# igormq/aes-lac-2018

Hardware: AMD Instinct MI355X
Metric: train frames/sec, DeepSpeech2 5xBiGRU-800 (higher is better)
Workload: dtype f32

## Files before the change

aes-lac-2018_amd/csrc/bn.hip:

```cpp
#include "ds2_common.h"

namespace {

constexpr int NPART = 64;

template <int MODE>
__global__ __launch_bounds__(256) void bn2d_reduce_kernel(const float* __restrict__ x, const float* __restrict__ dy,
                                                          const float* __restrict__ mean_invstd,
                                                          const float* __restrict__ gamma,
                                                          const float* __restrict__ beta, int B, int C, int inner,
                                                          double* __restrict__ part) {
    const int c = blockIdx.y, p = blockIdx.x, tid = threadIdx.x;
    const int chunks = (inner + 1023) / 1024;
    const int items = B * chunks;
    float mu = 0.f, is = 0.f, ga = 0.f, be = 0.f;
    if (MODE == 1) {
        mu = mean_invstd[c];
        is = mean_invstd[C + c];
        ga = gamma[c];
        be = beta[c];
    }
    float s0 = 0.f, s1 = 0.f;
    for (int it = p; it < items; it += NPART) {
        const int b = it / chunks, ch = it % chunks;
        const size_t base = ((size_t)b * C + c) * inner;
        const int i0 = ch * 1024;
#pragma unroll
        for (int u = 0; u < 4; ++u) {
            const int i = i0 + u * 256 + tid;
            if (i < inner) {
                const float v = x[base + i];
                if (MODE == 0) {
                    s0 += v;
                    s1 += v * v;
                } else {
                    const float xh = (v - mu) * is;
                    const float y = ga * xh + be;
                    const float g = (y > 0.f && y < 20.f) ? dy[base + i] : 0.f;
                    s0 += g;
                    s1 += g * xh;
                }
            }
        }
    }
    double d0 = wave_sum_d((double)s0), d1 = wave_sum_d((double)s1);
    __shared__ double sm[4][2];
    if ((tid & 63) == 0) {
        sm[tid >> 6][0] = d0;
        sm[tid >> 6][1] = d1;
    }
    __syncthreads();
    if (tid == 0) {
        part[((size_t)c * NPART + p) * 2 + 0] = sm[0][0] + sm[1][0] + sm[2][0] + sm[3][0];
        part[((size_t)c * NPART + p) * 2 + 1] = sm[0][1] + sm[1][1] + sm[2][1] + sm[3][1];
    }
}

template <int MODE>
__global__ __launch_bounds__(256) void bn2d_reduce_vec_kernel(const float* __restrict__ x, const float* __restrict__ dy,
                                                              const float* __restrict__ mean_invstd,
                                                              const float* __restrict__ gamma,
                                                              const float* __restrict__ beta, int B, int C, int inner,
                                                              double* __restrict__ part) {
    const int c = blockIdx.y, p = blockIdx.x, tid = threadIdx.x;
    const int chunks = (inner + 1023) / 1024;
    const int items = B * chunks;
    float mu = 0.f, is = 0.f, ga = 0.f, be = 0.f;
    if (MODE == 1) {
        mu = mean_invstd[c];
        is = mean_invstd[C + c];
        ga = gamma[c];
        be = beta[c];
    }
    float s0 = 0.f, s1 = 0.f;
    auto take = [&](float v, float g) {
        if (MODE == 0) {
            s0 += v;
            s1 += v * v;
        } else {
            const float xh = (v - mu) * is;
            const float y = ga * xh + be;
            const float gm = (y > 0.f && y < 20.f) ? g : 0.f;
            s0 += gm;
            s1 += gm * xh;
        }
    };
// ... 3 lines not shown
        const int h = min((int)((4 - (base & 3)) & 3), inner);
        const int nq = (inner - h) >> 2;
        const int q = ch * 256 + tid;
        if (q < nq) {
            const f32x4 v = *reinterpret_cast<const f32x4*>(x + base + h + 4 * (size_t)q);
            f32x4 g = {0.f, 0.f, 0.f, 0.f};
            if (MODE == 1) g = *reinterpret_cast<const f32x4*>(dy + base + h + 4 * (size_t)q);
#pragma unroll
            for (int e = 0; e < 4; ++e) take(v[e], g[e]);
        }
        if (ch == 0) {
            const int tail0 = h + 4 * nq, e = tid < 4 ? tid : tail0 + tid - 4;
            if ((tid < h) || (tid >= 4 && tid < 8 && e < inner)) take(x[base + e], MODE == 1 ? dy[base + e] : 0.f);
        }
    }
    double d0 = wave_sum_d((double)s0), d1 = wave_sum_d((double)s1);
    __shared__ double sm[4][2];
    if ((tid & 63) == 0) {
        sm[tid >> 6][0] = d0;
        sm[tid >> 6][1] = d1;
    }
    __syncthreads();
    if (tid == 0) {
        part[((size_t)c * NPART + p) * 2 + 0] = sm[0][0] + sm[1][0] + sm[2][0] + sm[3][0];
        part[((size_t)c * NPART + p) * 2 + 1] = sm[0][1] + sm[1][1] + sm[2][1] + sm[3][1];
    }
}

template <int MODE>
__global__ __launch_bounds__(256) void bn1d_reduce_kernel(const float* __restrict__ xa, const float* __restrict__ xb,
                                                          const float* __restrict__ dy,
                                                          const float* __restrict__ mean_invstd, int rows, int F,
                                                          double* __restrict__ part) {
    const int p = blockIdx.x, tid = threadIdx.x;
    const int col = blockIdx.y * 64 + (tid & 63), ry = tid >> 6;
    float mu = 0.f, is = 0.f;
    if (MODE == 1 && col < F) {
        mu = mean_invstd[col];
        is = mean_invstd[F + col];
    }
    float s0 = 0.f, s1 = 0.f;
    if (col < F) {
        for (int r = p * 4 + ry; r < rows; r += NPART * 4) {
            const size_t o = (size_t)r * F + col;
            float v = xa[o];
            if (xb) v += xb[o];
            if (MODE == 0) {
                s0 += v;
                s1 += v * v;
            } else {
                const float g = dy[o];
                s0 += g;
                s1 += g * (v - mu) * is;
            }
        }
    }
    __shared__ float sm[4][64][2];
    sm[ry][tid & 63][0] = s0;
    sm[ry][tid & 63][1] = s1;
    __syncthreads();
    if (ry == 0 && col < F) {
        const int l = tid & 63;
        const double d0 = (double)sm[0][l][0] + (double)sm[1][l][0] + (double)sm[2][l][0] + (double)sm[3][l][0];
        const double d1 = (double)sm[0][l][1] + (double)sm[1][l][1] + (double)sm[2][l][1] + (double)sm[3][l][1];
        part[((size_t)col * NPART + p) * 2 + 0] = d0;
        part[((size_t)col * NPART + p) * 2 + 1] = d1;
    }
}

__global__ __launch_bounds__(64) void bn_finalize_stats_kernel(const double* __restrict__ part, int C, double count,
                                                               float eps, float momentum, int use_running,
                                                               float* __restrict__ running_mean,
                                                               float* __restrict__ running_var,
                                                               float* __restrict__ mean_invstd) {
    const int c = blockIdx.x, lane = threadIdx.x;
    if (use_running) {
        if (lane == 0) {
            mean_invstd[c] = running_mean[c];
            mean_invstd[C + c] = (float)(1.0 / sqrt((double)running_var[c] + (double)eps));
        }
        return;
    }
    double s0 = part[((size_t)c * NPART + lane) * 2 + 0];
    double s1 = part[((size_t)c * NPART + lane) * 2 + 1];
    s0 = wave_sum_d(s0);
    s1 = wave_sum_d(s1);
    if (lane == 0) {
        const double mean = s0 / count;
        double var = s1 / count - mean * mean;
        if (var < 0.0) var = 0.0;
        mean_invstd[c] = (float)mean;
        mean_invstd[C + c] = (float)(1.0 / sqrt(var + (double)eps));
        if (running_mean) {
            const double unb = count > 1.0 ? var * count / (count - 1.0) : var;
            running_mean[c] = (float)((1.0 - momentum) * running_mean[c] + momentum * mean);
            running_var[c] = (float)((1.0 - momentum) * running_var[c] + momentum * unb);
        }
    }
}

__global__ __launch_bounds__(64) void bn_finalize_bwd_kernel(const double* __restrict__ part, int C, double count,
                                                             float* __restrict__ dgamma, float* __restrict__ dbeta,
                                                             float* __restrict__ coef) {
    const int c = blockIdx.x, lane = threadIdx.x;
    double s0 = part[((size_t)c * NPART + lane) * 2 + 0];
    double s1 = part[((size_t)c * NPART + lane) * 2 + 1];
    s0 = wave_sum_d(s0);
    s1 = wave_sum_d(s1);
    if (lane == 0) {
        dbeta[c] = (float)s0;
        dgamma[c] = (float)s1;
        coef[c] = (float)(s0 / count);
        coef[C + c] = (float)(s1 / count);
    }
}

__global__ __launch_bounds__(256) void bn2d_apply_kernel(const float* __restrict__ x,
                                                         const float* __restrict__ mean_invstd,
                                                         const float* __restrict__ gamma,
                                                         const float* __restrict__ beta, int C, int inner,
                                                         float* __restrict__ y) {
    const int bc = blockIdx.y, c = bc % C;
    const float sc = gamma[c] * mean_invstd[C + c];
    const float sh = beta[c] - mean_invstd[c] * sc;
    const size_t base = (size_t)bc * inner;
    for (int i = blockIdx.x * 256 + threadIdx.x; i < inner; i += gridDim.x * 256) {
        const float v = x[base + i] * sc + sh;
        y[base + i] = fminf(fmaxf(v, 0.f), 20.f);
    }
}

__global__ __launch_bounds__(256) void bn2d_apply_tbf_kernel(const float* __restrict__ x,
                                                             const float* __restrict__ mean_invstd,
                                                             const float* __restrict__ gamma,
                                                             const float* __restrict__ beta, int B, int C, int D,
                                                             int T, float* __restrict__ y) {
    __shared__ float tile[32][33];
// ... 155 lines not shown
            } else {
                const f32x4 g = dy[o];
                s0 += g;
                s1 += g * (v - mu) * is;
            }
        }
    }
    __shared__ f32x4 sm[4][64][2];
    sm[ry][tid & 63][0] = s0;
    sm[ry][tid & 63][1] = s1;
    __syncthreads();
    if (ry == 0 && cq < F4) {
        const int l = tid & 63;
#pragma unroll
        for (int e = 0; e < 4; ++e) {
            const double d0 = (double)sm[0][l][0][e] + (double)sm[1][l][0][e] + (double)sm[2][l][0][e] + (double)sm[3][l][0][e];
            const double d1 = (double)sm[0][l][1][e] + (double)sm[1][l][1][e] + (double)sm[2][l][1][e] + (double)sm[3][l][1][e];
            part[((size_t)(4 * cq + e) * NPART + p) * 2 + 0] = d0;
            part[((size_t)(4 * cq + e) * NPART + p) * 2 + 1] = d1;
        }
    }
}

__global__ __launch_bounds__(256) void bn1d_apply_vec_kernel(const f32x4* __restrict__ xa, const f32x4* __restrict__ xb,
                                                             const float* __restrict__ mean_invstd,
                                                             const float* __restrict__ gamma,
                                                             const float* __restrict__ beta, size_t n4, int F4,
                                                             f32x4* __restrict__ y) {
    const size_t stride = (size_t)gridDim.x * 256;
    for (size_t i = (size_t)blockIdx.x * 256 + threadIdx.x; i < n4; i += stride) {
        const int c = 4 * (int)(i % F4);
        f32x4 v = xa[i];
        if (xb) v += xb[i];
        const f32x4 sc = *reinterpret_cast<const f32x4*>(gamma + c) * *reinterpret_cast<const f32x4*>(mean_invstd + 4 * F4 + c);
        y[i] = (v - *reinterpret_cast<const f32x4*>(mean_invstd + c)) * sc + *reinterpret_cast<const f32x4*>(beta + c);
    }
}

__global__ __launch_bounds__(256) void bn1d_bwd_apply_vec_kernel(const f32x4* __restrict__ xa, const f32x4* __restrict__ xb,
                                                                 const f32x4* __restrict__ dy,
                                                                 const float* __restrict__ mean_invstd,
                                                                 const float* __restrict__ gamma,
                                                                 const float* __restrict__ coef, size_t n4, int F4,
                                                                 f32x4* __restrict__ dx) {
    const size_t stride = (size_t)gridDim.x * 256;
    const int F = 4 * F4;
    for (size_t i = (size_t)blockIdx.x * 256 + threadIdx.x; i < n4; i += stride) {
        const int c = 4 * (int)(i % F4);
        f32x4 v = xa[i];
        if (xb) v += xb[i];
        const f32x4 is = *reinterpret_cast<const f32x4*>(mean_invstd + F + c);
        const f32x4 xh = (v - *reinterpret_cast<const f32x4*>(mean_invstd + c)) * is;
        dx[i] = *reinterpret_cast<const f32x4*>(gamma + c) * is *
                (dy[i] - *reinterpret_cast<const f32x4*>(coef + c) - xh * *reinterpret_cast<const f32x4*>(coef + F + c));
    }
}

inline bool aligned16(const void* p) { return ((uintptr_t)p & 15) == 0; }
inline bool vec4_ok(int F, const void* a, const void* b, const void* c, const void* d) {
    return (F & 3) == 0 && ((((uintptr_t)a) | ((uintptr_t)b) | ((uintptr_t)c) | ((uintptr_t)d)) & 15) == 0;
}

inline int ew_blocks(size_t n) {
    size_t b = (n + 255) / 256;
    if (b > 4096) b = 4096;
    if (b < 1) b = 1;
    return (int)b;
}

}

extern "C" size_t ds2_bn_ws_bytes(int C) { return (size_t)C * NPART * 2 * sizeof(double) + (size_t)C * 2 * sizeof(float); }

extern "C" int ds2_bn2d_stats(const float* x, int B, int C, int inner, float eps, float momentum, int use_running,
                              float* running_mean, float* running_var, float* mean_invstd, void* ws, void* stream) {
    DS2_CHECK_ARG(x && mean_invstd && ws && B > 0 && C > 0 && inner > 0);
    DS2_CHECK_ARG(!use_running || (running_mean && running_var));
    hipStream_t st = (hipStream_t)stream;
    double* part = (double*)ws;
    if (!use_running) {
        if (aligned16(x))
            hipLaunchKernelGGL((bn2d_reduce_vec_kernel<0>), dim3(NPART, C), dim3(256), 0, st, x, nullptr, nullptr, nullptr,
                               nullptr, B, C, inner, part);
        else
            hipLaunchKernelGGL((bn2d_reduce_kernel<0>), dim3(NPART, C), dim3(256), 0, st, x, nullptr, nullptr, nullptr,
                               nullptr, B, C, inner, part);
    }
    hipLaunchKernelGGL(bn_finalize_stats_kernel, dim3(C), dim3(64), 0, st, part, C, (double)B * inner, eps, momentum,
                       use_running, running_mean, running_var, mean_invstd);
    DS2_CHECK_LAUNCH();
    return DS2_OK;
}

extern "C" int ds2_bn2d_apply_htanh(const float* x, const float* mean_invstd, const float* gamma, const float* beta,
                                    int B, int C, int D, int T, int layout_tbf, float* y, void* stream) {
    DS2_CHECK_ARG(x && mean_invstd && gamma && beta && y && B > 0 && C > 0 && D > 0 && T > 0);
    hipStream_t st = (hipStream_t)stream;
    if (layout_tbf) {
        DS2_CHECK_ARG(B <= 65535);
        dim3 grid(ds2_cdiv(T, 32), ds2_cdiv(C * D, 32), B);
        hipLaunchKernelGGL(bn2d_apply_tbf_kernel, grid, dim3(256), 0, st, x, mean_invstd, gamma, beta, B, C, D, T, y);
    } else {
        const int inner = D * T;
        if (aligned16(x) && aligned16(y)) {
            dim3 grid(min(ds2_cdiv(inner, 1024), 64), B * C);
            hipLaunchKernelGGL(bn2d_apply_vec_kernel, grid, dim3(256), 0, st, x, mean_invstd, gamma, beta, C, inner, y);
        } else {
            dim3 grid(min(ds2_cdiv(inner, 256), 64), B * C);
            hipLaunchKernelGGL(bn2d_apply_kernel, grid, dim3(256), 0, st, x, mean_invstd, gamma, beta, C, inner, y);
        }
    }
    DS2_CHECK_LAUNCH();
    return DS2_OK;
}

extern "C" int ds2_bn2d_htanh_bwd(const float* x, const float* dy, const float* mean_invstd, const float* gamma,
                                  const float* beta, int B, int C, int D, int T, float* dx, float* dgamma,
                                  float* dbeta, void* ws, void* stream) {
    DS2_CHECK_ARG(x && dy && mean_invstd && gamma && beta && dx && dgamma && dbeta && ws);
    DS2_CHECK_ARG(B > 0 && C > 0 && D > 0 && T > 0);
    hipStream_t st = (hipStream_t)stream;
    const int inner = D * T;
    double* part = (double*)ws;
    float* coef = (float*)(part + (size_t)C * NPART * 2);
    const bool vec = aligned16(x) && aligned16(dy) && aligned16(dx);
    if (vec)
        hipLaunchKernelGGL((bn2d_reduce_vec_kernel<1>), dim3(NPART, C), dim3(256), 0, st, x, dy, mean_invstd, gamma, beta,
                           B, C, inner, part);
    else
        hipLaunchKernelGGL((bn2d_reduce_kernel<1>), dim3(NPART, C), dim3(256), 0, st, x, dy, mean_invstd, gamma, beta, B,
                           C, inner, part);
    hipLaunchKernelGGL(bn_finalize_bwd_kernel, dim3(C), dim3(64), 0, st, part, C, (double)B * inner, dgamma, dbeta,
                       coef);
    if (vec) {
        dim3 grid(min(ds2_cdiv(inner, 1024), 64), B * C);
        hipLaunchKernelGGL(bn2d_bwd_apply_vec_kernel, grid, dim3(256), 0, st, x, dy, mean_invstd, gamma, beta, coef, C,
                           inner, dx);
    } else {
        dim3 grid(min(ds2_cdiv(inner, 256), 64), B * C);
        hipLaunchKernelGGL(bn2d_bwd_apply_kernel, grid, dim3(256), 0, st, x, dy, mean_invstd, gamma, beta, coef, C, inner,
                           dx);
    }
    DS2_CHECK_LAUNCH();
    return DS2_OK;
}

extern "C" int ds2_bn1d_stats(const float* xa, const float* xb, int rows, int F, float eps, float momentum,
                              int use_running, float* running_mean, float* running_var, float* mean_invstd, void* ws,
                              void* stream) {
    DS2_CHECK_ARG(xa && mean_invstd && ws && rows > 0 && F > 0);
    DS2_CHECK_ARG(!use_running || (running_mean && running_var));
    hipStream_t st = (hipStream_t)stream;
    double* part = (double*)ws;
    if (!use_running) {
        if (vec4_ok(F, xa, xb, nullptr, nullptr))
            hipLaunchKernelGGL((bn1d_reduce_vec_kernel<0>), dim3(NPART, ds2_cdiv(F / 4, 64)), dim3(256), 0, st,
                               (const f32x4*)xa, (const f32x4*)xb, nullptr, nullptr, rows, F, part);
        else
            hipLaunchKernelGGL((bn1d_reduce_kernel<0>), dim3(NPART, ds2_cdiv(F, 64)), dim3(256), 0, st, xa, xb, nullptr,
                               nullptr, rows, F, part);
    }
    hipLaunchKernelGGL(bn_finalize_stats_kernel, dim3(F), dim3(64), 0, st, part, F, (double)rows, eps, momentum,
                       use_running, running_mean, running_var, mean_invstd);
    DS2_CHECK_LAUNCH();
    return DS2_OK;
}

extern "C" int ds2_bn1d_apply(const float* xa, const float* xb, const float* mean_invstd, const float* gamma,
                              const float* beta, int rows, int F, float* y, void* stream) {
    DS2_CHECK_ARG(xa && mean_invstd && gamma && beta && y && rows > 0 && F > 0);
    const size_t n = (size_t)rows * F;
    if (vec4_ok(F, xa, xb, y, gamma) && vec4_ok(F, beta, mean_invstd, nullptr, nullptr))
        hipLaunchKernelGGL(bn1d_apply_vec_kernel, dim3(ew_blocks(n / 4)), dim3(256), 0, (hipStream_t)stream,
                           (const f32x4*)xa, (const f32x4*)xb, mean_invstd, gamma, beta, n / 4, F / 4, (f32x4*)y);
    else
        hipLaunchKernelGGL(bn1d_apply_kernel, dim3(ew_blocks(n)), dim3(256), 0, (hipStream_t)stream, xa, xb,
                           mean_invstd, gamma, beta, n, F, y);
    DS2_CHECK_LAUNCH();
    return DS2_OK;
}

extern "C" int ds2_bn1d_bwd(const float* xa, const float* xb, const float* dy, const float* mean_invstd,
                            const float* gamma, int rows, int F, float* dx, float* dgamma, float* dbeta, void* ws,
                            void* stream) {
    DS2_CHECK_ARG(xa && dy && mean_invstd && gamma && dx && dgamma && dbeta && ws && rows > 0 && F > 0);
    hipStream_t st = (hipStream_t)stream;
    double* part = (double*)ws;
    float* coef = (float*)(part + (size_t)F * NPART * 2);
    const bool vec = vec4_ok(F, xa, xb, dy, dx) && vec4_ok(F, gamma, mean_invstd, nullptr, nullptr);
    if (vec)
        hipLaunchKernelGGL((bn1d_reduce_vec_kernel<1>), dim3(NPART, ds2_cdiv(F / 4, 64)), dim3(256), 0, st,
                           (const f32x4*)xa, (const f32x4*)xb, (const f32x4*)dy, mean_invstd, rows, F, part);
    else
        hipLaunchKernelGGL((bn1d_reduce_kernel<1>), dim3(NPART, ds2_cdiv(F, 64)), dim3(256), 0, st, xa, xb, dy,
                           mean_invstd, rows, F, part);
    hipLaunchKernelGGL(bn_finalize_bwd_kernel, dim3(F), dim3(64), 0, st, part, F, (double)rows, dgamma, dbeta, coef);
    const size_t n = (size_t)rows * F;
    if (vec)
        hipLaunchKernelGGL(bn1d_bwd_apply_vec_kernel, dim3(ew_blocks(n / 4)), dim3(256), 0, st, (const f32x4*)xa,
                           (const f32x4*)xb, (const f32x4*)dy, mean_invstd, gamma, coef, n / 4, F / 4, (f32x4*)dx);
    else
        hipLaunchKernelGGL(bn1d_bwd_apply_kernel, dim3(ew_blocks(n)), dim3(256), 0, st, xa, xb, dy, mean_invstd, gamma,
                           coef, n, F, dx);
    DS2_CHECK_LAUNCH();
    return DS2_OK;
}
```

aes-lac-2018_amd/csrc/conv_split.hip:

```cpp
#include <stdlib.h>

#include <type_traits>

#include "split_bf16.h"

namespace {

constexpr int G_OOB = 0x7FFFFFF0;
constexpr int SPARE = 4;

struct GatherGeom {
    int M;
    int ngroups, npairs;
    int pair_stride, D;
    int row_len, rows_per_b;
    int a_base, a_b_stride, a_row_stride;
    int o_base, o_b_stride, o_row_stride, o_col_stride;
    int frows;
};

template <int NPROD, int NT>
__global__ __launch_bounds__(256, 2) void conv2_gather_kernel(const float* __restrict__ A, unsigned int a_bytes,
                                                              const int* __restrict__ tap_off,
                                                              const unsigned int* __restrict__ Wp, unsigned int w_bytes,
// ... 143 lines not shown
                    *c = acc[i][r] + bv;
            }
        }
}

__host__ __device__ inline int tap_groups(int nrows) { return 3 * (nrows / 2) + 2 * (nrows & 1); }
__device__ __forceinline__ void tap_slot(int nrows, int gq, int j, int& row, int& tap) {
    const int pairs = nrows >> 1;
    if (gq < 3 * pairs) {
        const int pr = gq / 3, w = gq - pr * 3;
        if (w < 2) {
            row = 2 * pr + w;
            tap = j;
        } else {
            row = 2 * pr + (j >> 2);
            tap = 8 + (j & 3);
        }
    } else {
        row = nrows - 1;
        tap = gq == 3 * pairs ? j : (j < 4 ? 8 + j : 11);
    }
    if (tap > 10) row = -1;
}
__global__ void conv2_split_prepare_kernel(const float* __restrict__ w, int mode, int nrows, int line, int spare,
                                           int* __restrict__ tap_off, unsigned int* __restrict__ Wp) {
    const int ng = tap_groups(nrows);
    const int i = blockIdx.x * 256 + threadIdx.x;
    if (i < (ng + spare) * 2) {
        const int gq = min(i >> 1, ng - 1);
        int row, tap;
        tap_slot(nrows, gq, (i & 1) * 4, row, tap);
        if (row < 0) tap_slot(nrows, gq, 0, row, tap);
        tap_off[i] = (mode == 0 ? row : 10 - row) * line + tap;
    }
    const int total = (16 * ng + spare) * 32 * 2 * 4;
    if (i >= total) return;
    const int jp = i & 3, half = (i >> 2) & 1, n = (i >> 3) & 31, step = i >> 8;
    const int cp = step / ng, gq = step - cp * ng;
    float v[2] = {0.f, 0.f};
    if (cp < 16) {
        const int c = 2 * cp + half;
#pragma unroll
        for (int e = 0; e < 2; ++e) {
            int row, tap;
            tap_slot(nrows, gq, jp * 2 + e, row, tap);
            if (row >= 0)
                v[e] = mode == 0 ? w[((n * 32 + c) * 21 + row) * 11 + tap]
                                 : w[((c * 32 + n) * 21 + 2 * row + (mode - 1)) * 11 + 10 - tap];
        }
    }
    unsigned int p1, p2, p3;
    split3(v[0], v[1], p1, p2, p3);
    unsigned int* dst = Wp + ((size_t)step * 3 * 32 * 16 + (n * 16 + half * 8 + jp * 2)) / 2;
    dst[0] = p1;
    dst[(32 * 16) / 2] = p2;
    dst[2 * (32 * 16) / 2] = p3;
}

__global__ __launch_bounds__(256) void conv2_pad_dout_kernel(const float* __restrict__ dy, int B, int T,
                                                             float* __restrict__ dyp) {
    const int TP = T + 20, nrows = B * 32 * 41;
    for (int r = blockIdx.x; r < nrows; r += gridDim.x) {
        const int bc = r / 41, fo = r - bc * 41 - 10;
        float* dst = dyp + (size_t)r * TP;
        if (fo < 0 || fo >= 21) {
            for (int tc = threadIdx.x; tc < TP; tc += 256) dst[tc] = 0.f;
        } else {
            const float* src = dy + ((size_t)bc * 21 + fo) * T - 10;
            for (int tc = threadIdx.x; tc < TP; tc += 256) dst[tc] = (tc >= 10 && tc < T + 10) ? src[tc] : 0.f;
        }
    }
}

int conv_split_mode() {
    const char* e = getenv("DS2_CONV_SPLIT");
    const int v = e ? atoi(e) : 6;
    return (v == 6 || v == 9) ? v : 0;
}

struct GatherPlan {
    int nt, tiles, per, nsplit;
};
GatherPlan plan_gather(int M, int nstep, bool may_split) {
    static const int force_ks = ds2_tune_env("DS2_CONV_SPLIT_KS") ? atoi(ds2_tune_env("DS2_CONV_SPLIT_KS")) : 0;
    static const int force_nt = ds2_tune_env("DS2_CONV_SPLIT_NT") ? atoi(ds2_tune_env("DS2_CONV_SPLIT_NT")) : 0;
    GatherPlan p;
    const int waves64 = ds2_cdiv(M, 64);
    p.nt = force_nt > 0 ? force_nt : (waves64 >= 1536 ? 2 : 1);
    p.tiles = ds2_cdiv(M, 128 * p.nt);
    const int waves = p.tiles * 4;
    const int ks = !may_split ? 1 : (force_ks > 0 ? force_ks : (waves >= 1024 ? 1 : (waves >= 512 ? 2 : 3)));
    p.per = ds2_cdiv(nstep, ks);
    p.nsplit = ds2_cdiv(nstep, p.per);
    return p;
// ... 65 lines not shown
    const unsigned int w_bytes = (unsigned int)((NP * NG + SPARE) * 3 * 32 * 16 * 2);
    launch_gather(mode, in, (unsigned int)a_bytes, tap_off, Wp, w_bytes, bias, out, o_elems, g, nstep, nullptr, st);
    return 0;
}

size_t ds2_conv2_dgrad_split_ws_floats(int B, int t1) {
    const size_t img0 = (size_t)(16 * tap_groups(11) + SPARE) * 3 * 32 * 16 / 2, img1 = (size_t)(16 * tap_groups(10) + SPARE) * 3 * 32 * 16 / 2;
    return 1024 + img0 + img1 + (size_t)B * 32 * 41 * (t1 + 10) + 64;
}

int ds2_conv2_dgrad_split(const float* d_out, const float* weight, int B, int t1, float* d_in, void* ws, hipStream_t st) {
    const int mode = conv_split_mode();
    if (mode == 0) return 1;
    const char* on = getenv("DS2_CONV_SPLIT_DGRAD");
    static const int dgrad_min = ds2_tune_env("DS2_CONV_SPLIT_DGRAD_MIN") ? atoi(ds2_tune_env("DS2_CONV_SPLIT_DGRAD_MIN")) : 1000;
    if (on ? on[0] != '1' : (long)B * t1 < dgrad_min) return 1;
    const int T = t1 - 10, TP = T + 20;
    const unsigned long long a_bytes = 4ull * B * 32 * 41 * TP, o_elems = 1ull * B * 32 * 61 * t1;
    if (a_bytes >= 0x7FFFFFF0ull || o_elems >= 0x7FFFFFF0ull) return 1;
    const size_t img0 = (size_t)(16 * tap_groups(11) + SPARE) * 3 * 32 * 16 / 2, img1 = (size_t)(16 * tap_groups(10) + SPARE) * 3 * 32 * 16 / 2;
    int* tab = reinterpret_cast<int*>(ws);
    unsigned int* Wp[2] = {reinterpret_cast<unsigned int*>(ws) + 1024, reinterpret_cast<unsigned int*>(ws) + 1024 + img0};
    float* dyp = reinterpret_cast<float*>(ws) + 1024 + img0 + img1;
    hipLaunchKernelGGL(conv2_pad_dout_kernel, dim3(B * 32 * 41 < 8192 ? B * 32 * 41 : 8192), dim3(256), 0, st, d_out, B, T, dyp);
    bool zeroed = false;
    for (int par = 0; par < 2; ++par)
        if (plan_gather(B * (par == 0 ? 31 : 30) * t1, 16 * tap_groups(par == 0 ? 11 : 10), true).nsplit > 1) zeroed = true;
    if (zeroed) (void)hipMemsetAsync(d_in, 0, o_elems * sizeof(float), st);
    GatherGeom gg[2];
    unsigned int wb[2];
    GatherPlan pp[2];
    for (int par = 0; par < 2; ++par) {
        const int nrows = par == 0 ? 11 : 10, ng = tap_groups(nrows), RH = par == 0 ? 31 : 30;
        const int prep = (16 * ng + SPARE) * 32 * 2 * 4;
        hipLaunchKernelGGL(conv2_split_prepare_kernel, dim3(ds2_cdiv(prep, 256)), dim3(256), 0, st, weight, 1 + par, nrows, TP,
                           SPARE, tab + 512 * par, Wp[par]);
        GatherGeom& g = gg[par];
        g.M = B * RH * t1;
        g.ngroups = ng;
        g.npairs = 16;
        g.pair_stride = 2 * 41 * TP;
        g.D = 41 * TP;
        g.row_len = t1;
        g.rows_per_b = RH;
        g.a_base = 0;
        g.a_b_stride = 32 * 41 * TP;
        g.a_row_stride = TP;
        g.o_base = par * t1;
        g.o_b_stride = 32 * 61 * t1;
        g.o_row_stride = 2 * t1;
        g.o_col_stride = 61 * t1;
        const char* rows_env = getenv("DS2_CONV_DGRAD_ROWS");
        const bool rows_off = rows_env && rows_env[0] == '0';
        pp[par] = plan_gather(g.M, 16 * ng, true);
        g.frows = (!rows_off && pp[par].nsplit == 1) ? nrows : 0;
        wb[par] = (unsigned int)((16 * ng + SPARE) * 3 * 32 * 16 * 2);
    }
    const char* merge_env = getenv("DS2_CONV_DGRAD_MERGE");
    const bool merge_off = merge_env && merge_env[0] == '0';
// ... 11 lines not shown
```

aes-lac-2018_amd/csrc/optim.hip:

```cpp
#include "ds2_common.h"

namespace {

constexpr int SS_BLOCKS = 1024;

__global__ __launch_bounds__(256) void sumsq_partial_kernel(const float* __restrict__ x, size_t n4, size_t n,
                                                            double* __restrict__ part) {
    float acc = 0.f;
    double dacc = 0.0;
    const size_t stride = (size_t)gridDim.x * 256;
    int cnt = 0;
    for (size_t i = (size_t)blockIdx.x * 256 + threadIdx.x; i < n4; i += stride) {
        const f32x4 v = reinterpret_cast<const f32x4*>(x)[i];
        acc += v[0] * v[0] + v[1] * v[1] + v[2] * v[2] + v[3] * v[3];
        if (++cnt == 64) {
            dacc += (double)acc;
            acc = 0.f;
            cnt = 0;
        }
    }
    if (blockIdx.x == 0)
        for (size_t i = n4 * 4 + threadIdx.x; i < n; i += 256) acc += x[i] * x[i];
    dacc += (double)acc;
    dacc = wave_sum_d(dacc);
    __shared__ double sm[4];
    if ((threadIdx.x & 63) == 0) sm[threadIdx.x >> 6] = dacc;
    __syncthreads();
    if (threadIdx.x == 0) part[blockIdx.x] = sm[0] + sm[1] + sm[2] + sm[3];
}

__global__ __launch_bounds__(256) void sumsq_final_kernel(const double* __restrict__ part, int nparts,
                                                          double* __restrict__ out) {
    double s = 0.0;
    for (int i = threadIdx.x; i < nparts; i += 256) s += part[i];
    s = wave_sum_d(s);
    __shared__ double sm[4];
    if ((threadIdx.x & 63) == 0) sm[threadIdx.x >> 6] = s;
    __syncthreads();
    if (threadIdx.x == 0) out[0] = sm[0] + sm[1] + sm[2] + sm[3];
}

__global__ __launch_bounds__(256) void clip_sgd_kernel(float* __restrict__ p, const float* __restrict__ g,
                                                       float* __restrict__ buf, size_t n4, size_t n,
                                                       const double* __restrict__ sumsq, float grad_scale,
                                                       float max_norm, float lr, float momentum, int first_step) {
    float coef = 1.f;
    if (sumsq) {
        const float total = (float)(sqrt(sumsq[0]) * (double)fabsf(grad_scale));
        const float c = max_norm / (total + 1e-6f);
        coef = c < 1.f ? c : 1.f;
    }
// ... 45 lines not shown

extern "C" int ds2_step_stats(const float* costs, int B, const double* sumsq, const uint32_t* const* err_words,
                              int n_err, double* out, void* stream) {
    DS2_CHECK_ARG(costs && out && B > 0 && n_err >= 0 && (n_err == 0 || err_words));
    hipLaunchKernelGGL(step_stats_kernel, dim3(1), dim3(64), 0, (hipStream_t)stream, costs, B, sumsq, err_words, n_err,
                       out);
    DS2_CHECK_LAUNCH();
    return DS2_OK;
}

extern "C" size_t ds2_sumsq_ws_bytes(size_t n) {
    (void)n;
    return SS_BLOCKS * sizeof(double);
}

extern "C" int ds2_sumsq(const float* x, size_t n, double* out, void* ws, void* stream) {
    DS2_CHECK_ARG(x && out && ws && n > 0);
    DS2_CHECK_ARG(((uintptr_t)x & 15) == 0);
    hipStream_t st = (hipStream_t)stream;
    const size_t n4 = n / 4;
    int blocks = (int)((n4 + 255) / 256);
    if (blocks > SS_BLOCKS) blocks = SS_BLOCKS;
    if (blocks < 1) blocks = 1;
    hipLaunchKernelGGL(sumsq_partial_kernel, dim3(blocks), dim3(256), 0, st, x, n4, n, (double*)ws);
    hipLaunchKernelGGL(sumsq_final_kernel, dim3(1), dim3(256), 0, st, (const double*)ws, blocks, out);
    DS2_CHECK_LAUNCH();
    return DS2_OK;
}

extern "C" int ds2_clip_sgd_nesterov(float* p, const float* g, float* buf, size_t n, const double* sumsq,
                                     float grad_scale, float max_norm, float lr, float momentum, int first_step,
                                     void* stream) {
    DS2_CHECK_ARG(p && g && buf && n > 0);
    DS2_CHECK_ARG((((uintptr_t)p | (uintptr_t)g | (uintptr_t)buf) & 15) == 0);
    const size_t n4 = n / 4;
    int blocks = (int)((n4 + 255) / 256);
    if (blocks > 2048) blocks = 2048;
    if (blocks < 1) blocks = 1;
    hipLaunchKernelGGL(clip_sgd_kernel, dim3(blocks), dim3(256), 0, (hipStream_t)stream, p, g, buf, n4, n, sumsq,
                       grad_scale, max_norm, lr, momentum, first_step);
    DS2_CHECK_LAUNCH();
    return DS2_OK;
}
```

Before: 561,400.

## Fold BN and sumsq finalize into reduce kernels via last-block tickets

Batch-norm reductions and the gradient sum-of-squares now use a global atomic ticket so that the last-arriving block performs the final reduction and finalize step, removing the separate finalize kernel launches. A vectorized 1D BN reduce kernel with a transposed partial layout is added. The conv2 dgrad padding and the two weight-prepare kernels are merged into one prologue launch. All three are on by default with env opt-outs. The cost is extra atomics and fences, and the ticket slots are shared state that could collide under concurrent streams.

```diff
diff --git a/aes-lac-2018_amd/csrc/bn.hip b/aes-lac-2018_amd/csrc/bn.hip
--- a/aes-lac-2018_amd/csrc/bn.hip
+++ b/aes-lac-2018_amd/csrc/bn.hip
@@ -1,15 +1,104 @@
 #include "ds2_common.h"
+#include <atomic>
 
 namespace {
 
 constexpr int NPART = 64;
 
+constexpr int FOLD_SLOTS = 256, FOLD_GROUPS = 256;
+__device__ unsigned int g_fold_ticket[FOLD_SLOTS * FOLD_GROUPS];
+
+struct FoldTail {
+    double count;
+    float eps, momentum;
+    float *running_mean, *running_var, *mean_invstd;
+    float *dgamma, *dbeta, *coef;
+    int ticket0;
+};
+
+__device__ __forceinline__ void fold_store(double* p, double v) {
+    __hip_atomic_store(p, v, __ATOMIC_RELAXED, __HIP_MEMORY_SCOPE_AGENT);
+}
+__device__ __forceinline__ double fold_load(const double* p) {
+    return __hip_atomic_load(p, __ATOMIC_RELAXED, __HIP_MEMORY_SCOPE_AGENT);
+}
+
+__device__ __forceinline__ bool fold_last_arriver(unsigned int* ticket) {
+    __shared__ unsigned int s_last;
+    asm volatile("s_waitcnt vmcnt(0)" ::: "memory");
+    __syncthreads();
+    if (threadIdx.x == 0) {
+        const unsigned int prev = __hip_atomic_fetch_add(ticket, 1u, __ATOMIC_RELAXED, __HIP_MEMORY_SCOPE_AGENT);
+        if (prev == NPART - 1) __hip_atomic_store(ticket, 0u, __ATOMIC_RELAXED, __HIP_MEMORY_SCOPE_AGENT);
+        s_last = prev == NPART - 1;
+    }
+    __syncthreads();
+    if (!s_last) return false;
+    __builtin_amdgcn_fence(__ATOMIC_ACQUIRE, "agent");
+    return true;
+}
+
+__device__ __forceinline__ double fold_tree(const double* part, size_t stride) {
+    double a[NPART / 2];
+#pragma unroll
+    for (int l = 0; l < NPART / 2; ++l) a[l] = fold_load(part + l * stride) + fold_load(part + (l + NPART / 2) * stride);
+#pragma unroll
+    for (int o = NPART / 4; o > 0; o >>= 1)
+#pragma unroll
+        for (int l = 0; l < o; ++l) a[l] += a[l + o];
+    return a[0];
+}
+
+__device__ __forceinline__ void finalize_stats(double s0, double s1, int c, int C, double count, float eps, float momentum,
+                                               float* running_mean, float* running_var, float* mean_invstd) {
+    const double mean = s0 / count;
+    double var = s1 / count - mean * mean;
+    if (var < 0.0) var = 0.0;
+    mean_invstd[c] = (float)mean;
+    mean_invstd[C + c] = (float)(1.0 / sqrt(var + (double)eps));
+    if (running_mean) {
+        const double unb = count > 1.0 ? var * count / (count - 1.0) : var;
+        running_mean[c] = (float)((1.0 - momentum) * running_mean[c] + momentum * mean);
+        running_var[c] = (float)((1.0 - momentum) * running_var[c] + momentum * unb);
+    }
+}
+__device__ __forceinline__ void finalize_bwd(double s0, double s1, int c, int C, double count, float* dgamma, float* dbeta,
+                                             float* coef) {
+    dbeta[c] = (float)s0;
+    dgamma[c] = (float)s1;
+    coef[c] = (float)(s0 / count);
+    coef[C + c] = (float)(s1 / count);
+}
 template <int MODE>
+__device__ __forceinline__ void fold_finalize(double s0, double s1, int c, int C, const FoldTail& t) {
+    if (MODE == 0) finalize_stats(s0, s1, c, C, t.count, t.eps, t.momentum, t.running_mean, t.running_var, t.mean_invstd);
+    else finalize_bwd(s0, s1, c, C, t.count, t.dgamma, t.dbeta, t.coef);
+}
+template <int MODE>
+__device__ __forceinline__ void fold_tail_2d(const double* part, int c, int C, const FoldTail& t) {
+    if (threadIdx.x >= 64) return;
+    const int lane = threadIdx.x;
+    double s0 = fold_load(part + ((size_t)c * NPART + lane) * 2 + 0);
+    double s1 = fold_load(part + ((size_t)c * NPART + lane) * 2 + 1);
+    s0 = wave_sum_d(s0);
+    s1 = wave_sum_d(s1);
+    if (lane == 0) fold_finalize<MODE>(s0, s1, c, C, t);
+}
+__device__ __forceinline__ size_t fold_part_1d(int p, int k, int col, int F) { return ((size_t)p * 2 + k) * F + col; }
+template <int MODE>
+__device__ __forceinline__ void fold_tail_1d(const double* part, int col, int F, const FoldTail& t) {
+    if (col >= F) return;
+    const double s0 = fold_tree(part + fold_part_1d(0, 0, col, F), (size_t)2 * F);
+    const double s1 = fold_tree(part + fold_part_1d(0, 1, col, F), (size_t)2 * F);
+    fold_finalize<MODE>(s0, s1, col, F, t);
+}
+
+template <int MODE, bool FOLD>
 __global__ __launch_bounds__(256) void bn2d_reduce_kernel(const float* __restrict__ x, const float* __restrict__ dy,
                                                           const float* __restrict__ mean_invstd,
                                                           const float* __restrict__ gamma,
                                                           const float* __restrict__ beta, int B, int C, int inner,
-                                                          double* __restrict__ part) {
+                                                          double* __restrict__ part, FoldTail ft) {
     const int c = blockIdx.y, p = blockIdx.x, tid = threadIdx.x;
     const int chunks = (inner + 1023) / 1024;
     const int items = B * chunks;
@@ -51,17 +140,24 @@
     }
     __syncthreads();
     if (tid == 0) {
-        part[((size_t)c * NPART + p) * 2 + 0] = sm[0][0] + sm[1][0] + sm[2][0] + sm[3][0];
-        part[((size_t)c * NPART + p) * 2 + 1] = sm[0][1] + sm[1][1] + sm[2][1] + sm[3][1];
-    }
-}
-
-template <int MODE>
+        const double d0s = sm[0][0] + sm[1][0] + sm[2][0] + sm[3][0], d1s = sm[0][1] + sm[1][1] + sm[2][1] + sm[3][1];
+        if (FOLD) {
+            fold_store(part + ((size_t)c * NPART + p) * 2 + 0, d0s);
+            fold_store(part + ((size_t)c * NPART + p) * 2 + 1, d1s);
+        } else {
+            part[((size_t)c * NPART + p) * 2 + 0] = d0s;
+            part[((size_t)c * NPART + p) * 2 + 1] = d1s;
+        }
+    }
+    if (FOLD && fold_last_arriver(g_fold_ticket + ft.ticket0 + c)) fold_tail_2d<MODE>(part, c, C, ft);
+}
+
+template <int MODE, bool FOLD>
 __global__ __launch_bounds__(256) void bn2d_reduce_vec_kernel(const float* __restrict__ x, const float* __restrict__ dy,
                                                               const float* __restrict__ mean_invstd,
                                                               const float* __restrict__ gamma,
                                                               const float* __restrict__ beta, int B, int C, int inner,
-                                                              double* __restrict__ part) {
+                                                              double* __restrict__ part, FoldTail ft) {
     const int c = blockIdx.y, p = blockIdx.x, tid = threadIdx.x;
     const int chunks = (inner + 1023) / 1024;
     const int items = B * chunks;
@@ -111,16 +207,23 @@
     }
     __syncthreads();
     if (tid == 0) {
-        part[((size_t)c * NPART + p) * 2 + 0] = sm[0][0] + sm[1][0] + sm[2][0] + sm[3][0];
-        part[((size_t)c * NPART + p) * 2 + 1] = sm[0][1] + sm[1][1] + sm[2][1] + sm[3][1];
-    }
-}
-
-template <int MODE>
+        const double d0s = sm[0][0] + sm[1][0] + sm[2][0] + sm[3][0], d1s = sm[0][1] + sm[1][1] + sm[2][1] + sm[3][1];
+        if (FOLD) {
+            fold_store(part + ((size_t)c * NPART + p) * 2 + 0, d0s);
+            fold_store(part + ((size_t)c * NPART + p) * 2 + 1, d1s);
+        } else {
+            part[((size_t)c * NPART + p) * 2 + 0] = d0s;
+            part[((size_t)c * NPART + p) * 2 + 1] = d1s;
+        }
+    }
+    if (FOLD && fold_last_arriver(g_fold_ticket + ft.ticket0 + c)) fold_tail_2d<MODE>(part, c, C, ft);
+}
+
+template <int MODE, bool FOLD>
 __global__ __launch_bounds__(256) void bn1d_reduce_kernel(const float* __restrict__ xa, const float* __restrict__ xb,
                                                           const float* __restrict__ dy,
                                                           const float* __restrict__ mean_invstd, int rows, int F,
-                                                          double* __restrict__ part) {
+                                                          double* __restrict__ part, FoldTail ft) {
     const int p = blockIdx.x, tid = threadIdx.x;
     const int col = blockIdx.y * 64 + (tid & 63), ry = tid >> 6;
     float mu = 0.f, is = 0.f;
@@ -152,9 +255,15 @@
         const int l = tid & 63;
         const double d0 = (double)sm[0][l][0] + (double)sm[1][l][0] + (double)sm[2][l][0] + (double)sm[3][l][0];
         const double d1 = (double)sm[0][l][1] + (double)sm[1][l][1] + (double)sm[2][l][1] + (double)sm[3][l][1];
-        part[((size_t)col * NPART + p) * 2 + 0] = d0;
-        part[((size_t)col * NPART + p) * 2 + 1] = d1;
-    }
+        if (FOLD) {
+            fold_store(part + fold_part_1d(p, 0, col, F), d0);
+            fold_store(part + fold_part_1d(p, 1, col, F), d1);
+        } else {
+            part[((size_t)col * NPART + p) * 2 + 0] = d0;
+            part[((size_t)col * NPART + p) * 2 + 1] = d1;
+        }
+    }
+    if (FOLD && fold_last_arriver(g_fold_ticket + ft.ticket0 + blockIdx.y) && tid < 64) fold_tail_1d<MODE>(part, blockIdx.y * 64 + tid, F, ft);
 }
 
 __global__ __launch_bounds__(64) void bn_finalize_stats_kernel(const double* __restrict__ part, int C, double count,
@@ -174,18 +283,7 @@
     double s1 = part[((size_t)c * NPART + lane) * 2 + 1];
     s0 = wave_sum_d(s0);
     s1 = wave_sum_d(s1);
-    if (lane == 0) {
-        const double mean = s0 / count;
-        double var = s1 / count - mean * mean;
-        if (var < 0.0) var = 0.0;
-        mean_invstd[c] = (float)mean;
-        mean_invstd[C + c] = (float)(1.0 / sqrt(var + (double)eps));
-        if (running_mean) {
-            const double unb = count > 1.0 ? var * count / (count - 1.0) : var;
-            running_mean[c] = (float)((1.0 - momentum) * running_mean[c] + momentum * mean);
-            running_var[c] = (float)((1.0 - momentum) * running_var[c] + momentum * unb);
-        }
-    }
+    if (lane == 0) finalize_stats(s0, s1, c, C, count, eps, momentum, running_mean, running_var, mean_invstd);
 }
 
 __global__ __launch_bounds__(64) void bn_finalize_bwd_kernel(const double* __restrict__ part, int C, double count,
@@ -196,12 +294,7 @@
     double s1 = part[((size_t)c * NPART + lane) * 2 + 1];
     s0 = wave_sum_d(s0);
     s1 = wave_sum_d(s1);
-    if (lane == 0) {
-        dbeta[c] = (float)s0;
-        dgamma[c] = (float)s1;
-        coef[c] = (float)(s0 / count);
-        coef[C + c] = (float)(s1 / count);
-    }
+    if (lane == 0) finalize_bwd(s0, s1, c, C, count, dgamma, dbeta, coef);
 }
 
 __global__ __launch_bounds__(256) void bn2d_apply_kernel(const float* __restrict__ x,
@@ -403,6 +496,82 @@
     }
 }
 
+constexpr int RQ = 32, RU = 4;
+template <int MODE, bool HAS_B>
+__global__ __launch_bounds__(4 * RQ) void bn1d_reduce_fold_vec_kernel(const f32x4* __restrict__ xa,
+                                                                      const f32x4* __restrict__ xb,
+                                                                      const f32x4* __restrict__ dy,
+                                                                      const float* __restrict__ mean_invstd, int rows, int F,
+                                                                      double* __restrict__ part, FoldTail ft) {
+    constexpr int STEP = NPART * 4;
+    const int p = blockIdx.x, tid = threadIdx.x;
+    const int F4 = F >> 2;
+    const int l = tid & (RQ - 1), cq = blockIdx.y * RQ + l, ry = tid / RQ;
+    f32x4 mu = {0.f, 0.f, 0.f, 0.f}, is = mu;
+    if (MODE == 1 && cq < F4) {
+        mu = *reinterpret_cast<const f32x4*>(mean_invstd + 4 * cq);
+        is = *reinterpret_cast<const f32x4*>(mean_invstd + F + 4 * cq);
+    }
+    f32x4 s0 = {0.f, 0.f, 0.f, 0.f}, s1 = s0;
+    if (cq < F4) {
+        f32x4 va[RU], vb[RU], vg[RU];
+        auto load = [&](int u, int r) {
+            const size_t o = (size_t)r * F4 + cq;
+            va[u] = xa[o];
+            if (HAS_B) vb[u] = xb[o];
+            if (MODE == 1) vg[u] = dy[o];
+        };
+        auto add = [&](int u, f32x4& a0, f32x4& a1) {
+            f32x4 v = va[u];
+            if (HAS_B) v += vb[u];
+            if (MODE == 0) {
+                a0 += v;
+                a1 += v * v;
+            } else {
+                const f32x4 g = vg[u];
+                a0 += g;
+                a1 += g * (v - mu) * is;
+            }
+        };
+        int r0 = p * 4 + ry;
+        for (; r0 + (RU - 1) * STEP < rows; r0 += RU * STEP) {
+#pragma unroll
+            for (int u = 0; u < RU; ++u) load(u, r0 + u * STEP);
+#pragma unroll
+            for (int u = 0; u < RU; ++u) add(u, s0, s1);
+        }
+        if (r0 < rows) {
+#pragma unroll
+            for (int u = 0; u < RU - 1; ++u) load(u, min(r0 + u * STEP, rows - 1));
+#pragma unroll
+            for (int u = 0; u < RU - 1; ++u) {
+                f32x4 t0 = s0, t1 = s1;
+                add(u, t0, t1);
+                const bool in = r0 + u * STEP < rows;
+#pragma unroll
+                for (int e = 0; e < 4; ++e) {
+                    s0[e] = in ? t0[e] : s0[e];
+                    s1[e] = in ? t1[e] : s1[e];
+                }
+            }
+        }
+    }
+    __shared__ f32x4 sm[4][RQ][2];
+    sm[ry][l][0] = s0;
+    sm[ry][l][1] = s1;
+    __syncthreads();
+    if (ry == 0 && cq < F4) {
+#pragma unroll
+        for (int e = 0; e < 4; ++e) {
+            const double d0 = (double)sm[0][l][0][e] + (double)sm[1][l][0][e] + (double)sm[2][l][0][e] + (double)sm[3][l][0][e];
+            const double d1 = (double)sm[0][l][1][e] + (double)sm[1][l][1][e] + (double)sm[2][l][1][e] + (double)sm[3][l][1][e];
+            fold_store(part + fold_part_1d(p, 0, 4 * cq + e, F), d0);
+            fold_store(part + fold_part_1d(p, 1, 4 * cq + e, F), d1);
+        }
+    }
+    if (fold_last_arriver(g_fold_ticket + ft.ticket0 + blockIdx.y)) fold_tail_1d<MODE>(part, blockIdx.y * 4 * RQ + tid, F, ft);
+}
+
 __global__ __launch_bounds__(256) void bn1d_apply_vec_kernel(const f32x4* __restrict__ xa, const f32x4* __restrict__ xb,
                                                              const float* __restrict__ mean_invstd,
                                                              const float* __restrict__ gamma,
@@ -449,6 +618,24 @@
     return (int)b;
 }
 
+#define DS2_BN1D_FOLD_GO(MODE_, DY_, MI_)                                                                               \
+    do {                                                                                                                \
+        const dim3 grid_(NPART, ds2_cdiv(F / 4, RQ));                                                                   \
+        if (xb)                                                                                                         \
+            hipLaunchKernelGGL((bn1d_reduce_fold_vec_kernel<MODE_, true>), grid_, dim3(4 * RQ), 0, st, (const f32x4*)xa, \
+                               (const f32x4*)xb, DY_, MI_, rows, F, part, ft);                                          \
+        else                                                                                                            \
+            hipLaunchKernelGGL((bn1d_reduce_fold_vec_kernel<MODE_, false>), grid_, dim3(4 * RQ), 0, st, (const f32x4*)xa, \
+                               (const f32x4*)xb, DY_, MI_, rows, F, part, ft);                                          \
+    } while (0)
+
+int fold_ticket0(int groups) {
+    static std::atomic<unsigned int> next{0};
+    const char* e = getenv("DS2_BN_FOLD");
+    if ((e && e[0] == '0') || groups > FOLD_GROUPS) return -1;
+    return (int)(next.fetch_add(1u, std::memory_order_relaxed) % FOLD_SLOTS) * FOLD_GROUPS;
+}
+
 }
 
 extern "C" size_t ds2_bn_ws_bytes(int C) { return (size_t)C * NPART * 2 * sizeof(double) + (size_t)C * 2 * sizeof(float); }
@@ -459,16 +646,30 @@
     DS2_CHECK_ARG(!use_running || (running_mean && running_var));
     hipStream_t st = (hipStream_t)stream;
     double* part = (double*)ws;
+    FoldTail ft = {};
+    ft.count = (double)B * inner;
+    ft.eps = eps;
+    ft.momentum = momentum;
+    ft.running_mean = running_mean;
+    ft.running_var = running_var;
+    ft.mean_invstd = mean_invstd;
+    ft.ticket0 = use_running ? -1 : fold_ticket0(C);
+    const bool fold = ft.ticket0 >= 0;
     if (!use_running) {
-        if (aligned16(x))
-            hipLaunchKernelGGL((bn2d_reduce_vec_kernel<0>), dim3(NPART, C), dim3(256), 0, st, x, nullptr, nullptr, nullptr,
-                               nullptr, B, C, inner, part);
-        else
-            hipLaunchKernelGGL((bn2d_reduce_kernel<0>), dim3(NPART, C), dim3(256), 0, st, x, nullptr, nullptr, nullptr,
-                               nullptr, B, C, inner, part);
-    }
-    hipLaunchKernelGGL(bn_finalize_stats_kernel, dim3(C), dim3(64), 0, st, part, C, (double)B * inner, eps, momentum,
-                       use_running, running_mean, running_var, mean_invstd);
+#define DS2_BN2D_GO(K_, FOLD_) \
+    hipLaunchKernelGGL((K_<0, FOLD_>), dim3(NPART, C), dim3(256), 0, st, x, nullptr, nullptr, nullptr, nullptr, B, C, inner, part, ft)
+        if (aligned16(x)) {
+            if (fold) DS2_BN2D_GO(bn2d_reduce_vec_kernel, true);
+            else DS2_BN2D_GO(bn2d_reduce_vec_kernel, false);
+        } else {
+            if (fold) DS2_BN2D_GO(bn2d_reduce_kernel, true);
+            else DS2_BN2D_GO(bn2d_reduce_kernel, false);
+        }
+#undef DS2_BN2D_GO
+    }
+    if (!fold)
+        hipLaunchKernelGGL(bn_finalize_stats_kernel, dim3(C), dim3(64), 0, st, part, C, (double)B * inner, eps, momentum,
+                           use_running, running_mean, running_var, mean_invstd);
     DS2_CHECK_LAUNCH();
     return DS2_OK;
 }
@@ -505,14 +706,26 @@
     double* part = (double*)ws;
     float* coef = (float*)(part + (size_t)C * NPART * 2);
     const bool vec = aligned16(x) && aligned16(dy) && aligned16(dx);
-    if (vec)
-        hipLaunchKernelGGL((bn2d_reduce_vec_kernel<1>), dim3(NPART, C), dim3(256), 0, st, x, dy, mean_invstd, gamma, beta,
-                           B, C, inner, part);
-    else
-        hipLaunchKernelGGL((bn2d_reduce_kernel<1>), dim3(NPART, C), dim3(256), 0, st, x, dy, mean_invstd, gamma, beta, B,
-                           C, inner, part);
-    hipLaunchKernelGGL(bn_finalize_bwd_kernel, dim3(C), dim3(64), 0, st, part, C, (double)B * inner, dgamma, dbeta,
-                       coef);
+    FoldTail ft = {};
+    ft.count = (double)B * inner;
+    ft.dgamma = dgamma;
+    ft.dbeta = dbeta;
+    ft.coef = coef;
+    ft.ticket0 = fold_ticket0(C);
+    const bool fold = ft.ticket0 >= 0;
+#define DS2_BN2D_GO(K_, FOLD_) \
+    hipLaunchKernelGGL((K_<1, FOLD_>), dim3(NPART, C), dim3(256), 0, st, x, dy, mean_invstd, gamma, beta, B, C, inner, part, ft)
+    if (vec) {
+        if (fold) DS2_BN2D_GO(bn2d_reduce_vec_kernel, true);
+        else DS2_BN2D_GO(bn2d_reduce_vec_kernel, false);
+    } else {
+        if (fold) DS2_BN2D_GO(bn2d_reduce_kernel, true);
+        else DS2_BN2D_GO(bn2d_reduce_kernel, false);
+    }
+#undef DS2_BN2D_GO
+    if (!fold)
+        hipLaunchKernelGGL(bn_finalize_bwd_kernel, dim3(C), dim3(64), 0, st, part, C, (double)B * inner, dgamma, dbeta,
+                           coef);
     if (vec) {
         dim3 grid(min(ds2_cdiv(inner, 1024), 64), B * C);
         hipLaunchKernelGGL(bn2d_bwd_apply_vec_kernel, grid, dim3(256), 0, st, x, dy, mean_invstd, gamma, beta, coef, C,
@@ -533,16 +746,32 @@
     DS2_CHECK_ARG(!use_running || (running_mean && running_var));
     hipStream_t st = (hipStream_t)stream;
     double* part = (double*)ws;
+    const bool vec = vec4_ok(F, xa, xb, nullptr, nullptr);
+    FoldTail ft = {};
+    ft.count = (double)rows;
+    ft.eps = eps;
+    ft.momentum = momentum;
+    ft.running_mean = running_mean;
+    ft.running_var = running_var;
+    ft.mean_invstd = mean_invstd;
+    ft.ticket0 = use_running ? -1 : fold_ticket0(vec ? ds2_cdiv(F / 4, RQ) : ds2_cdiv(F, 64));
+    const bool fold = ft.ticket0 >= 0;
     if (!use_running) {
-        if (vec4_ok(F, xa, xb, nullptr, nullptr))
+        if (vec && fold)
+            DS2_BN1D_FOLD_GO(0, nullptr, nullptr);
+        else if (vec)
             hipLaunchKernelGGL((bn1d_reduce_vec_kernel<0>), dim3(NPART, ds2_cdiv(F / 4, 64)), dim3(256), 0, st,
                                (const f32x4*)xa, (const f32x4*)xb, nullptr, nullptr, rows, F, part);
+        else if (fold)
+            hipLaunchKernelGGL((bn1d_reduce_kernel<0, true>), dim3(NPART, ds2_cdiv(F, 64)), dim3(256), 0, st, xa, xb, nullptr,
+                               nullptr, rows, F, part, ft);
         else
-            hipLaunchKernelGGL((bn1d_reduce_kernel<0>), dim3(NPART, ds2_cdiv(F, 64)), dim3(256), 0, st, xa, xb, nullptr,
-                               nullptr, rows, F, part);
-    }
-    hipLaunchKernelGGL(bn_finalize_stats_kernel, dim3(F), dim3(64), 0, st, part, F, (double)rows, eps, momentum,
-                       use_running, running_mean, running_var, mean_invstd);
+            hipLaunchKernelGGL((bn1d_reduce_kernel<0, false>), dim3(NPART, ds2_cdiv(F, 64)), dim3(256), 0, st, xa, xb, nullptr,
+                               nullptr, rows, F, part, ft);
+    }
+    if (!fold)
+        hipLaunchKernelGGL(bn_finalize_stats_kernel, dim3(F), dim3(64), 0, st, part, F, (double)rows, eps, momentum,
+                           use_running, running_mean, running_var, mean_invstd);
     DS2_CHECK_LAUNCH();
     return DS2_OK;
 }
@@ -569,13 +798,26 @@
     double* part = (double*)ws;
     float* coef = (float*)(part + (size_t)F * NPART * 2);
     const bool vec = vec4_ok(F, xa, xb, dy, dx) && vec4_ok(F, gamma, mean_invstd, nullptr, nullptr);
-    if (vec)
+    FoldTail ft = {};
+    ft.count = (double)rows;
+    ft.dgamma = dgamma;
+    ft.dbeta = dbeta;
+    ft.coef = coef;
+    ft.ticket0 = fold_ticket0(vec ? ds2_cdiv(F / 4, RQ) : ds2_cdiv(F, 64));
+    const bool fold = ft.ticket0 >= 0;
+    if (vec && fold)
+        DS2_BN1D_FOLD_GO(1, (const f32x4*)dy, mean_invstd);
+    else if (vec)
         hipLaunchKernelGGL((bn1d_reduce_vec_kernel<1>), dim3(NPART, ds2_cdiv(F / 4, 64)), dim3(256), 0, st,
                            (const f32x4*)xa, (const f32x4*)xb, (const f32x4*)dy, mean_invstd, rows, F, part);
+    else if (fold)
+        hipLaunchKernelGGL((bn1d_reduce_kernel<1, true>), dim3(NPART, ds2_cdiv(F, 64)), dim3(256), 0, st, xa, xb, dy,
+                           mean_invstd, rows, F, part, ft);
     else
-        hipLaunchKernelGGL((bn1d_reduce_kernel<1>), dim3(NPART, ds2_cdiv(F, 64)), dim3(256), 0, st, xa, xb, dy,
-                           mean_invstd, rows, F, part);
-    hipLaunchKernelGGL(bn_finalize_bwd_kernel, dim3(F), dim3(64), 0, st, part, F, (double)rows, dgamma, dbeta, coef);
+        hipLaunchKernelGGL((bn1d_reduce_kernel<1, false>), dim3(NPART, ds2_cdiv(F, 64)), dim3(256), 0, st, xa, xb, dy,
+                           mean_invstd, rows, F, part, ft);
+    if (!fold)
+        hipLaunchKernelGGL(bn_finalize_bwd_kernel, dim3(F), dim3(64), 0, st, part, F, (double)rows, dgamma, dbeta, coef);
     const size_t n = (size_t)rows * F;
     if (vec)
         hipLaunchKernelGGL(bn1d_bwd_apply_vec_kernel, dim3(ew_blocks(n / 4)), dim3(256), 0, st, (const f32x4*)xa,
diff --git a/aes-lac-2018_amd/csrc/conv_split.hip b/aes-lac-2018_amd/csrc/conv_split.hip
--- a/aes-lac-2018_amd/csrc/conv_split.hip
+++ b/aes-lac-2018_amd/csrc/conv_split.hip
@@ -189,10 +189,10 @@
     }
     if (tap > 10) row = -1;
 }
-__global__ void conv2_split_prepare_kernel(const float* __restrict__ w, int mode, int nrows, int line, int spare,
-                                           int* __restrict__ tap_off, unsigned int* __restrict__ Wp) {
+__device__ __forceinline__ void conv2_split_prepare(int block, const float* __restrict__ w, int mode, int nrows, int line,
+                                                    int spare, int* __restrict__ tap_off, unsigned int* __restrict__ Wp) {
     const int ng = tap_groups(nrows);
-    const int i = blockIdx.x * 256 + threadIdx.x;
+    const int i = block * 256 + threadIdx.x;
     if (i < (ng + spare) * 2) {
         const int gq = min(i >> 1, ng - 1);
         int row, tap;
@@ -223,11 +223,15 @@
     dst[(32 * 16) / 2] = p2;
     dst[2 * (32 * 16) / 2] = p3;
 }
-
-__global__ __launch_bounds__(256) void conv2_pad_dout_kernel(const float* __restrict__ dy, int B, int T,
-                                                             float* __restrict__ dyp) {
+__global__ void conv2_split_prepare_kernel(const float* __restrict__ w, int mode, int nrows, int line, int spare,
+                                           int* __restrict__ tap_off, unsigned int* __restrict__ Wp) {
+    conv2_split_prepare(blockIdx.x, w, mode, nrows, line, spare, tap_off, Wp);
+}
+
+__device__ __forceinline__ void conv2_pad_dout(int block, int nblocks, const float* __restrict__ dy, int B, int T,
+                                               float* __restrict__ dyp) {
     const int TP = T + 20, nrows = B * 32 * 41;
-    for (int r = blockIdx.x; r < nrows; r += gridDim.x) {
+    for (int r = block; r < nrows; r += nblocks) {
         const int bc = r / 41, fo = r - bc * 41 - 10;
         float* dst = dyp + (size_t)r * TP;
         if (fo < 0 || fo >= 21) {
@@ -237,6 +241,22 @@
             for (int tc = threadIdx.x; tc < TP; tc += 256) dst[tc] = (tc >= 10 && tc < T + 10) ? src[tc] : 0.f;
         }
     }
+}
+__global__ __launch_bounds__(256) void conv2_pad_dout_kernel(const float* __restrict__ dy, int B, int T,
+                                                             float* __restrict__ dyp) {
+    conv2_pad_dout(blockIdx.x, gridDim.x, dy, B, T, dyp);
+}
+
+__global__ __launch_bounds__(256) void conv2_dgrad_prologue_kernel(const float* __restrict__ dy, int B, int T,
+                                                                   float* __restrict__ dyp, int pad_blocks,
+                                                                   const float* __restrict__ w, int line, int spare,
+                                                                   int prep0, int* __restrict__ tab,
+                                                                   unsigned int* __restrict__ Wp0,
+                                                                   unsigned int* __restrict__ Wp1) {
+    const int b = blockIdx.x;
+    if (b < pad_blocks) conv2_pad_dout(b, pad_blocks, dy, B, T, dyp);
+    else if (b < pad_blocks + prep0) conv2_split_prepare(b - pad_blocks, w, 1, 11, line, spare, tab, Wp0);
+    else conv2_split_prepare(b - pad_blocks - prep0, w, 2, 10, line, spare, tab + 512, Wp1);
 }
 
 int conv_split_mode() {
@@ -348,7 +368,17 @@
     int* tab = reinterpret_cast<int*>(ws);
     unsigned int* Wp[2] = {reinterpret_cast<unsigned int*>(ws) + 1024, reinterpret_cast<unsigned int*>(ws) + 1024 + img0};
     float* dyp = reinterpret_cast<float*>(ws) + 1024 + img0 + img1;
-    hipLaunchKernelGGL(conv2_pad_dout_kernel, dim3(B * 32 * 41 < 8192 ? B * 32 * 41 : 8192), dim3(256), 0, st, d_out, B, T, dyp);
+    const char* pro_env = getenv("DS2_CONV_DGRAD_PROLOGUE");
+    const bool prologue = !(pro_env && pro_env[0] == '0');
+    const int pad_blocks = B * 32 * 41 < 8192 ? B * 32 * 41 : 8192;
+    if (prologue) {
+        const int prep0 = ds2_cdiv((16 * tap_groups(11) + SPARE) * 32 * 2 * 4, 256);
+        const int prep1 = ds2_cdiv((16 * tap_groups(10) + SPARE) * 32 * 2 * 4, 256);
+        hipLaunchKernelGGL(conv2_dgrad_prologue_kernel, dim3(pad_blocks + prep0 + prep1), dim3(256), 0, st, d_out, B, T, dyp,
+                           pad_blocks, weight, TP, SPARE, prep0, tab, Wp[0], Wp[1]);
+    } else {
+        hipLaunchKernelGGL(conv2_pad_dout_kernel, dim3(pad_blocks), dim3(256), 0, st, d_out, B, T, dyp);
+    }
     bool zeroed = false;
     for (int par = 0; par < 2; ++par)
         if (plan_gather(B * (par == 0 ? 31 : 30) * t1, 16 * tap_groups(par == 0 ? 11 : 10), true).nsplit > 1) zeroed = true;
@@ -359,8 +389,9 @@
     for (int par = 0; par < 2; ++par) {
         const int nrows = par == 0 ? 11 : 10, ng = tap_groups(nrows), RH = par == 0 ? 31 : 30;
         const int prep = (16 * ng + SPARE) * 32 * 2 * 4;
-        hipLaunchKernelGGL(conv2_split_prepare_kernel, dim3(ds2_cdiv(prep, 256)), dim3(256), 0, st, weight, 1 + par, nrows, TP,
-                           SPARE, tab + 512 * par, Wp[par]);
+        if (!prologue)
+            hipLaunchKernelGGL(conv2_split_prepare_kernel, dim3(ds2_cdiv(prep, 256)), dim3(256), 0, st, weight, 1 + par, nrows,
+                               TP, SPARE, tab + 512 * par, Wp[par]);
         GatherGeom& g = gg[par];
         g.M = B * RH * t1;
         g.ngroups = ng;
diff --git a/aes-lac-2018_amd/csrc/optim.hip b/aes-lac-2018_amd/csrc/optim.hip
--- a/aes-lac-2018_amd/csrc/optim.hip
+++ b/aes-lac-2018_amd/csrc/optim.hip
@@ -1,11 +1,16 @@
 #include "ds2_common.h"
+#include <atomic>
 
 namespace {
 
 constexpr int SS_BLOCKS = 1024;
 
+constexpr int SS_SLOTS = 64;
+__device__ unsigned int g_ss_ticket[SS_SLOTS];
+
+template <bool FOLD>
 __global__ __launch_bounds__(256) void sumsq_partial_kernel(const float* __restrict__ x, size_t n4, size_t n,
-                                                            double* __restrict__ part) {
+                                                            double* __restrict__ part, int slot, double* __restrict__ out) {
     float acc = 0.f;
     double dacc = 0.0;
     const size_t stride = (size_t)gridDim.x * 256;
@@ -26,7 +31,28 @@
     __shared__ double sm[4];
     if ((threadIdx.x & 63) == 0) sm[threadIdx.x >> 6] = dacc;
     __syncthreads();
-    if (threadIdx.x == 0) part[blockIdx.x] = sm[0] + sm[1] + sm[2] + sm[3];
+    if (!FOLD) {
+        if (threadIdx.x == 0) part[blockIdx.x] = sm[0] + sm[1] + sm[2] + sm[3];
+        return;
+    }
+    __shared__ unsigned int s_last;
+    if (threadIdx.x == 0) {
+        __hip_atomic_store(part + blockIdx.x, sm[0] + sm[1] + sm[2] + sm[3], __ATOMIC_RELAXED, __HIP_MEMORY_SCOPE_AGENT);
+        asm volatile("s_waitcnt vmcnt(0)" ::: "memory");
+        const unsigned int prev = __hip_atomic_fetch_add(g_ss_ticket + slot, 1u, __ATOMIC_RELAXED, __HIP_MEMORY_SCOPE_AGENT);
+        if (prev == gridDim.x - 1) __hip_atomic_store(g_ss_ticket + slot, 0u, __ATOMIC_RELAXED, __HIP_MEMORY_SCOPE_AGENT);
+        s_last = prev == gridDim.x - 1;
+    }
+    __syncthreads();
+    if (!s_last) return;
+    __builtin_amdgcn_fence(__ATOMIC_ACQUIRE, "agent");
+    double s = 0.0;
+    for (int i = threadIdx.x; i < (int)gridDim.x; i += 256)
+        s += __hip_atomic_load(part + i, __ATOMIC_RELAXED, __HIP_MEMORY_SCOPE_AGENT);
+    s = wave_sum_d(s);
+    if ((threadIdx.x & 63) == 0) sm[threadIdx.x >> 6] = s;
+    __syncthreads();
+    if (threadIdx.x == 0) out[0] = sm[0] + sm[1] + sm[2] + sm[3];
 }
 
 __global__ __launch_bounds__(256) void sumsq_final_kernel(const double* __restrict__ part, int nparts,
@@ -118,8 +144,15 @@
     int blocks = (int)((n4 + 255) / 256);
     if (blocks > SS_BLOCKS) blocks = SS_BLOCKS;
     if (blocks < 1) blocks = 1;
-    hipLaunchKernelGGL(sumsq_partial_kernel, dim3(blocks), dim3(256), 0, st, x, n4, n, (double*)ws);
-    hipLaunchKernelGGL(sumsq_final_kernel, dim3(1), dim3(256), 0, st, (const double*)ws, blocks, out);
+    static std::atomic<unsigned int> next{0};
+    const char* e = getenv("DS2_SUMSQ_FOLD");
+    if (e && e[0] == '0') {
+        hipLaunchKernelGGL(sumsq_partial_kernel<false>, dim3(blocks), dim3(256), 0, st, x, n4, n, (double*)ws, 0, out);
+        hipLaunchKernelGGL(sumsq_final_kernel, dim3(1), dim3(256), 0, st, (const double*)ws, blocks, out);
+    } else {
+        const int slot = (int)(next.fetch_add(1u, std::memory_order_relaxed) % SS_SLOTS);
+        hipLaunchKernelGGL(sumsq_partial_kernel<true>, dim3(blocks), dim3(256), 0, st, x, n4, n, (double*)ws, slot, out);
+    }
     DS2_CHECK_LAUNCH();
     return DS2_OK;
 }
```

New measurement: 560,400. No clear change (-0.2%).
